# TimingSpace/MVOScaleRecovery

Measured on AMD Instinct MI355X. Metric: frames/sec scale-recovery, KITTI-00 flow (~2k feats/frame), 1/2/4/8 GPU, higher is better.
Workload: dtype f64

## Files before the change

### mvoscalerecovery_amd/csrc/mvosr_kernels.hip

```cpp
#include <hip/hip_runtime.h>
#include <math.h>
#include <stdint.h>
#include <stdlib.h>
#include <string.h>

#include "../../include/mvosr.h"
#include "mvosr_device.hpp"
#include "mvosr_host.hpp"

namespace mvosr {

#ifdef MVOSR_STAMPS
#define MVOSR_STAMP(i) do { if (threadIdx.x == 0 && stamps) stamps[i] = __builtin_amdgcn_s_memtime(); } while (0)
#define MVOSR_STAMP_DECL unsigned long long stamps[12] = {0,0,0,0,0,0,0,0,0,0,0,0};
#define MVOSR_STAMP_ARG , unsigned long long *stamps = nullptr
#define MVOSR_STAMP_PASS , stamps
#define MVOSR_RSTAMP(i) do { if (stamps) stamps[i] = __builtin_amdgcn_s_memtime(); } while (0)
#else
#define MVOSR_RSTAMP(i) do {} while (0)
#define MVOSR_STAMP(i) do {} while (0)
#define MVOSR_STAMP_DECL
#define MVOSR_STAMP_ARG
#define MVOSR_STAMP_PASS
#endif
// ... 519 lines not shown
    double res = 0.0;
    for (int c0 = 0; c0 < n_steep; c0 += kNpBufSize) {
        const int m = min(kNpBufSize, n_steep - c0);
        int k = 0;
        np_pairwise_leaves(m, [&](int lo, int len, bool is_leaf) {
            if (is_leaf) { if (k % B == tid) leaf[k] = np_leaf_sum(hs + c0 + lo, len, 0.0, false); ++k; }
        });
        __threadfence_block();
        __syncthreads();
        if (tid == 0) {
            double val[kNpDepth + 1];
            int vp = 0, kk = 0;
            np_pairwise_leaves(m, [&](int, int, bool is_leaf) {
                if (is_leaf) val[vp++] = leaf[kk++];
                else { const double r = val[--vp], l = val[--vp]; val[vp++] = l + r; }
            });
            *slot = c0 == 0 ? val[0] : *slot + val[0];
        }
        __syncthreads();
    }
    res = *slot;
    __syncthreads();
    return (0.0 + res) / (double)n_steep;
}

struct LdsFetch {
    const double2 *P; const double *Y; int n_valid;
    __device__ __forceinline__ bool operator()(const TriIds q, double &x0, double &y0, double &z0, double &x1, double &y1, double &z1,
                                               double &x2, double &y2, double &z2) const {
        if ((unsigned)q.a >= (unsigned)n_valid || (unsigned)q.b >= (unsigned)n_valid || (unsigned)q.c >= (unsigned)n_valid) return false;
        const double2 p0 = p_ld(P, Y, q.a), p1 = p_ld(P, Y, q.b), p2 = p_ld(P, Y, q.c);
        x0 = p0.x; z0 = p0.y; x1 = p1.x; z1 = p1.y; x2 = p2.x; z2 = p2.y;
        y0 = Y[q.a]; y1 = Y[q.b]; y2 = Y[q.c];
        return true;
    }
};

constexpr double kLevelGuard = 1e-12;

template <int WAVES, int MODE, int FW = 1>
__device__ __forceinline__ SelectResult phase_select(const Smem &s, int n_valid, const int32_t *tri2, int64_t t2_begin,
                                                     int t2_count, TriChunk<WAVES * kWave> &tc, PitchTest pt,
                                                     double *g_normals, double *g_pitch, double *g_heights, int bad_in,
                                                     double *scratch, int scratch_cap, int dbg = 0 MVOSR_STAMP_ARG) {
    constexpr int B = WAVES * kWave;
    constexpr bool FULL = MODE == MODE_FULL;
    const int tid = threadIdx.x;
    unsigned long long flat = 0ull;
    unsigned long long flat_hi = 0ull;
    double hsum = 0.0, hcnt = 0.0, habs = 0.0;
    int npitch = 0, singular = 0, bad = 0;
    int undecided = 0;
    if (t2_count > 64 * FW * B) { bad = 1; t2_count = 0; }
    auto test_triangle = [&](int t, int kk, const TriIds q) {
    if ((unsigned)q.a >= (unsigned)n_valid || (unsigned)q.b >= (unsigned)n_valid || (unsigned)q.c >= (unsigned)n_valid) { bad = 1; return; }
    const double2 p0 = p_ld(s.P, s.Y, q.a), p1 = p_ld(s.P, s.Y, q.b), p2 = p_ld(s.P, s.Y, q.c);
    const double y0 = s.Y[q.a], y1 = s.Y[q.b], y2 = s.Y[q.c];
    const double x0 = p0.x, z0 = p0.y, x1 = p1.x, z1 = p1.y, x2 = p2.x, z2 = p2.y;
    const double h = MODE == MODE_HOT ? (y0 + y1) + y2 : div3((y0 + y1) + y2);
    const int r = classify_triangle<FULL>(x0, y0, z0, x1, y1, z1, x2, y2, z2, h, pt, g_normals, g_pitch, g_heights, t2_begin + t);
    const bool is_flat = r & 1, is_steep = r & 2;
    if (r & 4) singular = 1;
    if constexpr (MODE == MODE_HOT) { if (r & 8) undecided = 1; }
    if (is_steep) { hsum += h; hcnt += 1.0; if constexpr (MODE == MODE_HOT) habs += fabs(h); }
    if (is_flat) {
        if (FW == 1 || kk < 64) flat |= 1ull << (kk & 63); else flat_hi |= 1ull << (kk & 63);
        ++npitch;
    }
    };
    const int t2c = (dbg & 2) ? 0 : t2_count;
    TriChunk<B> tn;
    for (int base = 0; base < t2c; base += kTC * B) {
        const bool more = base + kTC * B < t2c;
        if (more) tn.load(tri2, t2_begin, t2_count, base + kTC * B, tid);
#pragma unroll
        for (int k = 0; k < kTC; ++k) {
            const int t = base + k * B + tid;
            if (t < t2c) test_triangle(t, base / B + k, tc.q[k]);
        }
        if (more) tc = tn;
    }
    const int t2d = (dbg & 4) ? 0 : t2_count;
    const bool in_regs = t2_count <= kTC * B;
    if (!in_regs && t2d > 0) tc.template load<true>(tri2, t2_begin, t2_count, 0, tid);
    if constexpr (MODE == MODE_HOT) block_sum3<WAVES>(hsum, hcnt, habs, s.red + R_SEL_H * 2 * WAVES, s.red + R_SEL_ABS * 2 * WAVES);
    else block_sum2<WAVES>(hsum, hcnt, s.red + R_SEL_H * 2 * WAVES);
    MVOSR_STAMP(4);
    SelectResult r;
    double hl = hsum / hcnt;
    const double guard = kLevelGuard * (habs / hcnt);
    if constexpr (MODE != MODE_HOT) {
        if (scratch && (int)hcnt + kNpMaxLeaves <= scratch_cap)
            hl = exact_height_level_block<WAVES, FULL>(tri2 + 3 * t2_begin, t2_count, (int)hcnt, pt, LdsFetch{s.P, s.Y, n_valid}, nullptr,
                                                       scratch, s.misc + M_WCNT, s.red + R_MISC * 2 * WAVES);
        else
            hl = exact_height_level<FULL>(tri2 + 3 * t2_begin, t2_count, (int)hcnt, pt, LdsFetch{s.P, s.Y, n_valid});
    }
    int ntv = 0, near = undecided;
    auto mark_triangle = [&](int kk, int qa, int qb, int qc) {
        const unsigned long long fw = (FW == 1 || kk < 64) ? flat : flat_hi;
        if (!((fw >> (kk & 63)) & 1ull)) return;
        const double y0 = s.Y[qa], y1 = s.Y[qb], y2 = s.Y[qc];
        const double h = MODE == MODE_HOT ? (y0 + y1) + y2 : div3((y0 + y1) + y2);
        if constexpr (MODE == MODE_HOT) { if (fabs(h - hl) <= guard) near = 1; }
        if (h > hl) {
            ++ntv;
            atomicOr(&s.sel[qa >> 5], 1u << (qa & 31));
            atomicOr(&s.sel[qb >> 5], 1u << (qb & 31));
            atomicOr(&s.sel[qc >> 5], 1u << (qc & 31));
        }
    };
    for (int base = 0; base < t2d; base += kTC * B) {
        const bool more = base + kTC * B < t2d;
        if (more) tn.template load<true>(tri2, t2_begin, t2_count, base + kTC * B, tid);
#pragma unroll
        for (int k = 0; k < kTC; ++k) {
            if (base + k * B + tid < t2d) mark_triangle(base / B + k, tc.q[k].a, tc.q[k].b, tc.q[k].c);
        }
        if (more) tc = tn;
    }
    bad |= bad_in;
    int sn = singular | (near << 16);
    block_sum4i<WAVES>(npitch, ntv, sn, bad, s.red + R_SEL_CNT * 2 * WAVES);
    singular = sn & 0xFFFF;
    r.near = sn >> 16;
    MVOSR_STAMP(5);
    r.height_level = MODE == MODE_HOT ? hl / 3.0 : hl;
    r.n_steep = (int)hcnt;
    r.n_pitch = npitch; r.n_tri_valid = ntv; r.singular = singular; r.bad = bad;
    return r;
}

struct RoadResult {
    double height;
    int status;
    int n_sel, n_kept, n_modes, mode_left, mode_right;
    double mean, std, skew, median;
};

__device__ __forceinline__ bool dropped_by_single(double y, int bin, const Bits192 &single, int first_single) {
    bool d = false;
#pragma unroll
    for (int dk = -1; dk <= 1; ++dk) {
        const int k = bin + dk;
        const bool is_single = (k >= 0) && (k < kBins) && single.test_lane(max(k, 0));
        const double r = bin_edge(k + 1);
        const double lo = r - 0.1;
        const bool in = (k == first_single) ? (y >= lo && y <= r) : (y > lo && y <= r);
        d |= is_single && in;
    }
    return d;
}

#ifndef MVOSR_ROAD_RC
#define MVOSR_ROAD_RC 20
#endif
constexpr int kRoadRC = MVOSR_ROAD_RC;
constexpr int kDropStride = 32;
constexpr int kRoadWaves = 4;
constexpr int kTrash = 175;
constexpr int kStPending = -1;
constexpr int kStRedo = -2;
static_assert(kStRedo == MVOSR_ST_REDO, "include/mvosr.h");
constexpr int kMaxVoteRows = 32765;

struct RoadArgs {
    mvosr_params P;
    const int64_t *off;
    const int32_t *cnt;
    const double *y;
    double *scratch;
    const double *height_level;
    mvosr_outputs o;
    int64_t first_frame, n_frames;
    int pending_only;
    int32_t *level_redo;
    const int32_t *list;
    int wide;
    const uint8_t *listed_mask = nullptr;
};

__device__ __forceinline__ int bin_of_table(double y, const double2 *edges) {
    if (!(y >= 0.0 && y <= bin_edge(kBins))) return -1;
    int k = min((int)(y * 10.0), kBins - 1);
    const double2 e = edges[k];
    k += (k < kBins - 1 && y >= e.y) ? 1 : 0;
    k -= (y < e.x) ? 1 : 0;
    return k;
}

template <int RC, int WW = 1>
__device__ __forceinline__ RoadResult road_wave(int *hist, int *nearflag, uint16_t *slots, uint8_t *dropb, const double2 *edges,
                                                const double *yv_all, double *scratch,
                                                int Mall, double height_level, const mvosr_params &P, int32_t *g_hist, bool exact_stats,
                                                int part_lo, int part_hi, double *part, int *np_stack MVOSR_STAMP_ARG) {
    const int lane = lane_id();
    RoadResult R;
    R.height = nan(""); R.status = MVOSR_ST_MODE; R.n_sel = Mall; R.n_kept = 0; R.n_modes = 0; R.mode_left = -1; R.mode_right = -1;
    R.mean = R.std = R.skew = R.median = nan("");
    if (Mall == 0) { R.status = MVOSR_ST_NO_FLAT; return R; }
    const double *yv = yv_all + (part_hi > part_lo ? part_lo : 0);
    const int M = part_hi - part_lo;
    if (WW == 1 || wave_id() == 0) {
#pragma unroll
        for (int c = 0; c < 3; ++c) { const int b = lane + 64 * c; if (b < 176) hist[b] = 0; }
    }
    if constexpr (WW > 1) __syncthreads();

    double yc[RC];
    int binc[RC];
    const int nfull = M / kWave;
    const unsigned valid = (nfull >= RC) ? (unsigned)((1ull << RC) - 1ull)
                                              : (((1u << nfull) - 1u) | ((lane < M - nfull * kWave ? 1u : 0u) << nfull));
#pragma unroll
    for (int k = 0; k < RC; ++k) {
        const int i = max(min(k * kWave + lane, M - 1), 0);
        yc[k] = yv[i];
    }
#pragma unroll
    for (int k = 0; k < RC; ++k) {
        const double y = yc[k];
        const bool inr = ((valid >> k) & 1u) && (y >= 0.0) && (y <= bin_edge(kBins));
        const int g = inr ? min((int)(y * 10.0), kBins - 1) : 0;
        const double2 e = edges[g];
        int bin = g + ((g < kBins - 1 && y >= e.y) ? 1 : 0) - ((y < e.x) ? 1 : 0);
        bin = inr ? bin : kTrash;
        atomicAdd(&hist[bin], 1);
        binc[k] = bin;
    }
    constexpr int kLongUnroll = 8;
    for (int i0 = RC * kWave + lane; i0 < M; i0 += kLongUnroll * kWave) {
        double yl[kLongUnroll];
#pragma unroll
        for (int j = 0; j < kLongUnroll; ++j) yl[j] = yv[max(min(i0 + j * kWave, M - 1), 0)];
#pragma unroll
        for (int j = 0; j < kLongUnroll; ++j) {
            const int bin = (i0 + j * kWave < M) ? bin_of_table(yl[j], edges) : -1;
            if (bin >= 0) atomicAdd(&hist[bin], 1);
        }
    }
    MVOSR_RSTAMP(2);
    if constexpr (WW > 1) __syncthreads();
    int hraw[3], hz[3];
    Bits192 single, modes, mins;
    int mx = 0, mn = 0x7fffffff;
#pragma unroll
    for (int c = 0; c < 3; ++c) {
        const int b = lane + 64 * c;
        hraw[c] = (b < kBins) ? hist[b] : 0;
        hz[c] = (hraw[c] == 1) ? 0 : hraw[c];
        single.w[c] = __ballot(b < kBins && hraw[c] == 1);
        mx = max(mx, hz[c]);
        if (b < kBins) mn = min(mn, hz[c]);
    }
    mx = wave_max(mx);
    mn = wave_min(mn);
    if (g_hist && (WW == 1 || wave_id() == 0)) {
#pragma unroll
        for (int c = 0; c < 3; ++c) { const int b = lane + 64 * c; if (b < kBins) { g_hist[b] = hraw[c]; g_hist[kBins + b] = hz[c]; } }
    }
    MVOSR_RSTAMP(3);
    const int first_single = single.lowest_from(0);
    Bits192 near;
    near.w[0] = single.w[0] | (single.w[0] << 1) | (single.w[0] >> 1) | (single.w[1] << 63);
    near.w[1] = single.w[1] | (single.w[1] << 1) | (single.w[1] >> 1) | (single.w[0] >> 63) | (single.w[2] << 63);
    near.w[2] = single.w[2] | (single.w[2] << 1) | (single.w[2] >> 1) | (single.w[1] >> 63);
#pragma unroll
    for (int c = 0; c < 3; ++c) { const int b = lane + 64 * c; if (b < 176) nearflag[b] = (b < kBins) ? (int)((near.w[c] >> lane) & 1ull) : 0; }
    const bool have_modes = mx > P.mode_min;

    unsigned kept = valid;
    {
        uint4 zero; zero.x = zero.y = zero.z = zero.w = 0u;
        reinterpret_cast<uint4 *>(dropb)[2 * lane] = zero;
        if (RC > 16) reinterpret_cast<uint4 *>(dropb)[2 * lane + 1] = zero;
        int ns = 0;
#pragma unroll
        for (int k = 0; k < RC; ++k) {
            const bool sus = nearflag[binc[k]] != 0;
            const unsigned long long m = __ballot(sus);
            if (sus) slots[ns + __popcll(m & ((1ull << lane) - 1ull))] = (uint16_t)(k * kWave + lane);
            ns += __popcll(m);
        }
        for (int i = lane; i < ns; i += kWave) {
            const int e = slots[i];
            const double y = yv[e];
            if (dropped_by_single(y, bin_of_table(y, edges), single, first_single)) dropb[(e & (kWave - 1)) * kDropStride + (e >> 6)] = 1;
        }
        if (ns > 0) {
#pragma unroll
            for (int j = 0; j < (RC + 15) / 16; ++j) {
                const uint4 d = reinterpret_cast<const uint4 *>(dropb)[2 * lane + j];
#pragma unroll
                for (int k = 16 * j; k < RC && k < 16 * j + 16; ++k) {
                    const int kk = k & 15;
                    const unsigned w = (kk >> 2) == 0 ? d.x : ((kk >> 2) == 1 ? d.y : ((kk >> 2) == 2 ? d.z : d.w));
                    if ((w >> (8 * (kk & 3))) & 0xFFu) kept &= ~(1u << k);
                }
            }
        }
    }
    double sum = 0.0;
#pragma unroll
    for (int k = 0; k < RC; ++k) sum += ((kept >> k) & 1u) ? yc[k] : 0.0;
    double cntd = (double)__popc(kept);
    for (int i0 = RC * kWave + lane; i0 < M; i0 += kLongUnroll * kWave) {
        double yl[kLongUnroll];
#pragma unroll
        for (int j = 0; j < kLongUnroll; ++j) yl[j] = yv[max(min(i0 + j * kWave, M - 1), 0)];
#pragma unroll
        for (int j = 0; j < kLongUnroll; ++j) {
            if (i0 + j * kWave >= M) continue;
            const double y = yl[j];
            const int bin = bin_of_table(y, edges);
            if (bin >= 0 && nearflag[bin] && dropped_by_single(y, bin, single, first_single)) continue;
            sum += y; cntd += 1.0;
        }
    }
    sum = wave_sum(sum);
    cntd = wave_sum(cntd);
    if constexpr (WW > 1) {
        if (lane == 0) { part[2 * wave_id()] = sum; part[2 * wave_id() + 1] = cntd; }
        __syncthreads();
        sum = 0.0; cntd = 0.0;
#pragma unroll
        for (int i = 0; i < WW; ++i) { sum += part[2 * i]; cntd += part[2 * i + 1]; }
        __syncthreads();
    }
    MVOSR_RSTAMP(4);
    const int nkept = (int)cntd;
    R.n_kept = nkept;

    auto pack_kept = [&]() {
        int nlist = 0;
#pragma unroll 1
        for (int i0 = 0; i0 < Mall; i0 += kWave) {
            const int i = i0 + lane;
            bool keep = false;
            double y = 0.0;
            if (i < Mall) {
                y = yv_all[i];
                const int bin = bin_of_table(y, edges);
                keep = !(bin >= 0 && nearflag[bin] && dropped_by_single(y, bin, single, first_single));
            }
            const unsigned long long m = __ballot(keep);
            if (keep) scratch[nlist + __popcll(m & ((1ull << lane) - 1ull))] = y;
            nlist += __popcll(m);
        }
        return nlist;
    };

    if (!have_modes) {
        if constexpr (WW > 1) { if (wave_id() != 0) return R; }
        if (nkept == 0) { R.height = height_level; R.status = MVOSR_ST_LEVEL; return R; }
        pack_kept();
        __threadfence_block();
        const int klo = (nkept - 1) >> 1, khi = nkept >> 1;
        double mlo = 0.0, mhi = 0.0;
        int flo = 0, fhi = 0;
        for (int i = lane; i < nkept; i += kWave) {
            const double yi = scratch[i];
            int rank = 0;
            for (int j = 0; j < nkept; ++j) {
                const double yj = scratch[j];
                rank += (yj < yi) || (yj == yi && j < i);
            }
            if (rank == klo) { mlo = yi; flo = 1; }
            if (rank == khi) { mhi = yi; fhi = 1; }
        }
        const unsigned long long blo = __ballot(flo), bhi = __ballot(fhi);
        mlo = readlane_d(mlo, (int)__ffsll((long long)blo) - 1);
        mhi = readlane_d(mhi, (int)__ffsll((long long)bhi) - 1);
        R.median = (klo == khi) ? mlo : (mlo + mhi) / 2.0;
        R.height = R.median; R.status = MVOSR_ST_MEDIAN;
        return R;
    }

    const double mean = sum / cntd;
    double ss = 0.0;
#pragma unroll
    for (int k = 0; k < RC; ++k) {
        const double d = ((kept >> k) & 1u) ? yc[k] - mean : 0.0;
        ss += d * d;
    }
    for (int i0 = RC * kWave + lane; i0 < M; i0 += kLongUnroll * kWave) {
        double yl[kLongUnroll];
#pragma unroll
        for (int j = 0; j < kLongUnroll; ++j) yl[j] = yv[max(min(i0 + j * kWave, M - 1), 0)];
#pragma unroll
        for (int j = 0; j < kLongUnroll; ++j) {
            if (i0 + j * kWave >= M) continue;
            const double y = yl[j];
            const int bin = bin_of_table(y, edges);
            if (bin >= 0 && nearflag[bin] && dropped_by_single(y, bin, single, first_single)) continue;
            const double d = y - mean;
            ss += d * d;
        }
    }
    ss = wave_sum(ss);
    if constexpr (WW > 1) {
        if (lane == 0) part[wave_id()] = ss;
        __syncthreads();
        if (wave_id() != 0) return R;
        ss = 0.0;
#pragma unroll
        for (int i = 0; i < WW; ++i) ss += part[i];
    }
    MVOSR_RSTAMP(5);

#pragma unroll
    for (int c = 0; c < 3; ++c) {
        const int b = lane + 64 * c;
        bool is_mode = false, is_min = false;
        if (b < kBins) {
            const int h = hz[c];
            if (b == 0 || b == kBins - 1) {
                is_mode = (h == mx);
                is_min = (h == mn);
            } else {
                const int lraw = hist[b - 1], rraw = hist[b + 1];
                const int hl_ = (lraw == 1) ? 0 : lraw, hr_ = (rraw == 1) ? 0 : rraw;
                is_mode = (h >= hl_) && (h >= hr_) && ((double)h >= P.mode_rel * (double)mx) && (h >= P.mode_min);
                is_min = (h <= hl_) && (h <= hr_) && !((h == hr_) && (h == hl_));
            }
        }
        modes.w[c] = __ballot(is_mode);
        mins.w[c] = __ballot(is_min);
    }
    R.n_modes = modes.runs();
    const int i_last = modes.highest_below(kBins);
    int i_first = i_last;
    while (i_first > 0 && modes.test(i_first - 1)) --i_first;
    const int ml = i_first + 1, mr = i_last + 1;
    R.mode_left = ml; R.mode_right = mr;
    const double mode = (double)(ml + mr) / 2.0;
    const int il = mins.highest_below(ml);
    if (il < 0) { R.status = MVOSR_ST_ERR_LEFT; return R; }
    const int ir = mins.lowest_from(mr);
    if (ir < 0) { R.status = MVOSR_ST_ERR_RIGHT; return R; }
    const double right = bin_edge(ir + 1);
    double mean_o = mean;
    double sd = sqrt(ss / cntd);
    {
        const double var = ss / cntd, rms = sqrt(mean * mean + var);
        const double margin = fabs((mean - mode / 10.0) - P.skew_threshold * sd);
        const double bound = 1e-11 * (rms + sd) + 1e-22 * rms * rms / sd;
        if (!(margin > bound) || exact_stats) {
            const int nl = pack_kept();
            __threadfence_block();
            mean_o = np_pairwise_sum_cold(scratch, nl, 0.0, 0, np_stack) / (double)nl;
            sd = sqrt(np_pairwise_sum_cold(scratch, nl, mean_o, 1, np_stack) / (double)nl);
        }
    }
    const double skew = (mean_o - mode / 10.0) / sd;
    R.mean = mean_o; R.std = sd; R.skew = skew;
    if (skew > P.skew_threshold) { R.height = right; R.status = MVOSR_ST_RIGHT; }
    else { R.height = mode / 10.0; R.status = MVOSR_ST_MODE; }
    return R;
}

#ifndef MVOSR_ROAD_MINW
#define MVOSR_ROAD_MINW 1
#endif
template <bool LIST, int WW = 1>
__global__ __launch_bounds__(kRoadWaves *kWave, (LIST ? 1 : 4)) void road_model_kernel(const RoadArgs a) {
    static_assert(kRoadRC >= 16 && kRoadRC <= kDropStride, "verdict bytes per lane; the keep masks are 32 bits");
    static_assert(WW == 1 || (WW == kRoadWaves && !LIST), "wide variant: the whole workgroup on one frame");
    __shared__ int hist_all[kRoadWaves][2][176];
    __shared__ double2 edges[kBins + 1];
    __shared__ uint16_t slots_all[kRoadWaves][kRoadRC * kWave];
    __shared__ __attribute__((aligned(16))) uint8_t drop_all[kRoadWaves][kDropStride * kWave];
    __shared__ double part[2 * kRoadWaves];
    __shared__ __attribute__((aligned(8))) int np_stack_all[kRoadWaves][kNpStackInts];
    for (int k = threadIdx.x; k < kBins; k += kRoadWaves * kWave) { double2 e; e.x = bin_edge(k); e.y = bin_edge(k + 1); edges[k] = e; }
    __syncthreads();
    const int64_t slot = WW > 1 ? (int64_t)blockIdx.x : (int64_t)blockIdx.x * kRoadWaves + wave_id();
    auto one_frame = [&](const int64_t f) {
    if (a.pending_only && a.o.status[f] != kStPending) return;
    MVOSR_STAMP_DECL
    MVOSR_RSTAMP(0);
    const int M = a.cnt[f];
    const int64_t off = a.off[f];
    const double hl = a.height_level ? a.height_level[f] : nan("");
    MVOSR_RSTAMP(1);
    int *h0 = hist_all[WW > 1 ? 0 : wave_id()][0], *h1 = hist_all[wave_id()][1];
    int32_t *gh = a.o.hist ? a.o.hist + f * 2 * kBins : nullptr;
    const bool ex = a.o.stats != nullptr;
    int lo = 0, hi = M;
    if constexpr (WW > 1) {
        const int q = ((M + WW * kWave - 1) / (WW * kWave)) * kWave;
        lo = min(M, wave_id() * q);
        hi = min(M, lo + q);
    }
    const int Mp = hi - lo;
#define MVOSR_ROAD_CALL(RC_) road_wave<RC_, WW>(h0, h1, slots_all[wave_id()], drop_all[wave_id()], edges, a.y + off, a.scratch + off, M, hl, a.P, gh, ex, lo, hi, part, np_stack_all[wave_id()] MVOSR_STAMP_PASS)
    const RoadResult R = (Mp <= 4 * kWave) ? MVOSR_ROAD_CALL(4)
                       : (Mp <= 8 * kWave) ? MVOSR_ROAD_CALL(8)
                       : (Mp <= 12 * kWave) ? MVOSR_ROAD_CALL(12)
                       : (kRoadRC == 16 || Mp <= 16 * kWave) ? MVOSR_ROAD_CALL(16)
                                          : MVOSR_ROAD_CALL(kRoadRC);
#undef MVOSR_ROAD_CALL
    MVOSR_RSTAMP(6);
#ifdef MVOSR_STAMPS
    if (lane_id() == 0 && a.o.hist) { unsigned long long *d = reinterpret_cast<unsigned long long *>(a.o.hist + f * 2 * kBins) + 16; for (int i = 0; i < 8; ++i) d[i] = stamps[i]; }
#endif
    if (WW > 1 && wave_id() != 0) return;
    if (R.status == MVOSR_ST_LEVEL && a.level_redo) {
        if (lane_id() == 0) {
            if (!(a.listed_mask && a.listed_mask[f])) a.level_redo[1 + atomicAdd(a.level_redo, 1)] = (int32_t)f;
            a.o.status[f] = kStRedo;
        }
        return;
    }
    if (lane_id() == 0) {
        double height = nan(""), raw = nan("");
        if (R.status == MVOSR_ST_NO_FLAT) raw = a.P.absolute_reference / hl;
        else if (R.status <= MVOSR_ST_LEVEL) { height = R.height; raw = a.P.absolute_reference / height; }
        a.o.raw_scale[f] = raw; a.o.height[f] = height; a.o.status[f] = R.status;
        if (!a.pending_only && a.o.height_level) a.o.height_level[f] = hl;
        if (a.o.counts) {
            int32_t *c = a.o.counts + f * MVOSR_N_COUNTS;
            if (!a.pending_only) { c[MVOSR_CNT_VALID] = M; c[MVOSR_CNT_TRI_PITCH] = 0; c[MVOSR_CNT_TRI_VALID] = 0; }
            c[MVOSR_CNT_SELECTED] = R.n_sel; c[MVOSR_CNT_KEPT] = R.n_kept; c[MVOSR_CNT_MODES] = R.n_modes;
            c[MVOSR_CNT_MODE_LEFT] = R.mode_left; c[MVOSR_CNT_MODE_RIGHT] = R.mode_right;
        }
        if (a.o.stats) { double *st = a.o.stats + 4 * f; st[0] = R.mean; st[1] = R.std; st[2] = R.skew; st[3] = R.median; }
    }
    };
    if constexpr (LIST) {
        const int64_t n_todo = (int64_t)a.list[0];
        for (int64_t it = slot; it < n_todo; it += (int64_t)gridDim.x * kRoadWaves) one_frame((int64_t)a.list[1 + it]);
    } else {
        if (slot < a.n_frames) one_frame(a.first_frame + slot);
    }
}

struct KArgs {
    mvosr_params P;
    mvosr_batch b;
    mvosr_outputs o;
    PitchTest pt;
    int64_t first_frame;
    const double *height_level_in;
    int debug_skip;
    int32_t *redo;
    int redo_pass;
    double *ysel;
    int32_t *nsel;
    const int32_t *cls_list;
    const int32_t *cls_cnt;
};

__device__ __forceinline__ void write_counts(const KArgs &a, int64_t f, int nvalid, int npitch, int ntv, const RoadResult &R) {
    if (!a.o.counts) return;
    int32_t *c = a.o.counts + f * MVOSR_N_COUNTS;
    c[MVOSR_CNT_VALID] = nvalid; c[MVOSR_CNT_TRI_PITCH] = npitch; c[MVOSR_CNT_TRI_VALID] = ntv;
    c[MVOSR_CNT_SELECTED] = R.n_sel; c[MVOSR_CNT_KEPT] = R.n_kept; c[MVOSR_CNT_MODES] = R.n_modes;
    c[MVOSR_CNT_MODE_LEFT] = R.mode_left; c[MVOSR_CNT_MODE_RIGHT] = R.mode_right;
}

__device__ __forceinline__ bool early_frame_exit(const KArgs &a, int64_t f, int n, int t2n) {
    const bool too_few = n == 3;
    const bool oversize = n > a.b.max_feat;
    if (!(n <= 2 || too_few || t2n <= 0 || oversize)) return false;
    if (threadIdx.x == 0) {
        RoadResult R;
        R.n_sel = R.n_kept = R.n_modes = 0; R.mode_left = R.mode_right = -1;
        a.o.raw_scale[f] = nan(""); a.o.height[f] = nan(""); a.o.height_level[f] = nan("");
        a.o.status[f] = oversize ? MVOSR_ST_ERR_MASK : (too_few ? MVOSR_ST_TOO_FEW : MVOSR_ST_ERR_EMPTY);
        a.nsel[f] = 0;
        write_counts(a, f, too_few ? n : 0, 0, 0, R);
    }
    return true;
}

template <int BW, int MODE>
__device__ __forceinline__ void frame_tail(const KArgs &a, const Smem &s, int64_t f, int64_t off, int nvalid, bool refused,
                                           SelectResult &S, RoadResult &R) {
    constexpr int B = BW * kWave;
    const int tid = threadIdx.x;
    int status = kStPending;
    double raw = nan("");
    int nsel = 0;
    if (refused || S.bad) {
        status = MVOSR_ST_ERR_MASK;
    } else if (S.singular) {
        status = MVOSR_ST_ERR_SINGULAR;
    } else {
        const int w = wave_id(), lane = lane_id();
        const int per = ((nvalid + B - 1) / B) * kWave;
        const int begin = w * per, end = min(nvalid, begin + per);
        int cnt = 0;
        for (int j0 = begin; j0 < end; j0 += kWave) {
            const int j = j0 + lane;
            const bool sel = (j < end) && ((s.sel[j >> 5] >> (j & 31)) & 1u);
            if (a.o.selected && j < end) a.o.selected[off + j] = (uint8_t)sel;
            cnt += __popcll(__ballot(sel));
        }
        if (lane == 0) s.misc[M_WCNT + w] = cnt;
        __syncthreads();
        int base = 0;
#pragma unroll
        for (int i = 0; i < BW; ++i) { const int c = s.misc[M_WCNT + i]; if (i < w) base += c; nsel += c; }
        if constexpr (MODE == MODE_HOT) {
            if (S.near || nsel == 0) {
                if (tid == 0) { a.redo[1 + atomicAdd(a.redo, 1)] = (int32_t)f; a.o.status[f] = kStRedo; a.nsel[f] = 0; }
                return;
            }
        }
        double *dst = a.ysel + off;
        for (int j0 = begin; j0 < end; j0 += kWave) {
            const int j = j0 + lane;
            const bool sel = (j < end) && ((s.sel[j >> 5] >> (j & 31)) & 1u);
            const unsigned long long m = __ballot(sel);
            if (sel) dst[base + __popcll(m & ((1ull << lane) - 1ull))] = s.Y[j];
            base += __popcll(m);
        }
        if (nsel == 0) { status = MVOSR_ST_NO_FLAT; raw = a.P.absolute_reference / S.height_level; }
    }
    if (tid == 0) {
        a.o.raw_scale[f] = raw;
        a.o.height[f] = nan("");
        a.o.height_level[f] = S.height_level;
        a.o.status[f] = status;
        a.nsel[f] = nsel;
        R.n_sel = nsel;
        write_counts(a, f, nvalid, S.n_pitch, S.n_tri_valid, R);
        if (a.o.stats) { double *st = a.o.stats + 4 * f; st[0] = st[1] = st[2] = st[3] = nan(""); }
    }
}

template <int MODE, bool LIST, class Body>
__device__ __forceinline__ void for_frames(const KArgs &a, Body body) {
    if constexpr (MODE == MODE_EXACT) {
        if (a.redo_pass) {
            const int count = a.redo[0];
            for (int i = blockIdx.x; i < count; i += gridDim.x) {
                body((int64_t)a.redo[1 + i]);
                __syncthreads();
            }
            return;
        }
    }
    if constexpr (LIST) {
        if ((int)blockIdx.x < *a.cls_cnt) body((int64_t)a.cls_list[blockIdx.x]);
        return;
    }
    body(a.first_frame + blockIdx.x);
}

#ifndef MVOSR_MINW
#define MVOSR_MINW 1
// ... 1290 lines not shown
        if ((rc = launch_append_mask(ctx, ka, n_launch, false))) return rc;
        if (standin && (rc = standin_rows(ka.redo))) return rc;
        if ((rc = dense ? launch_scale_dense(ctx, ka, n_launch, kModeExactList, false) : dispatch_scale(ctx, ka, waves, n_launch, kModeExactList))) return rc;
        ra.first_frame = first_frame; ra.n_frames = n_launch; ra.list = ka.redo;
        ra.wide = (dense && !(debug_skip_env() & 256)) ? 1 : 0;
        return launch_road(ctx, ra, ctx_stream(ctx));
    }
    const bool fold = mode == MODE_HOT && (hot_only || (!(debug_skip_env() & 16) && !(debug_skip_env() & 512)));
    if (by_class) {
        if ((rc = launch_scale_classes(ctx, ka, n_launch))) return rc;
        if (!hot_only && (rc = launch_append_mask(ctx, ka, n_launch, true))) return rc;
        if (!fold && (rc = dispatch_scale(ctx, ka, waves, n_launch, kModeExactList))) return rc;
    } else {
        g_defer_exact = fold;
        g_hot_only = hot_only;
        rc = dense ? launch_scale_dense(ctx, ka, n_launch, mode, false) : dispatch_scale(ctx, ka, waves, n_launch, mode);
        g_defer_exact = false;
        g_hot_only = false;
        if (rc) return rc;
    }
    if (pev && (ee = hipEventRecord(pev[1], ctx_stream(ctx))) != hipSuccess) return set_hip_error("hipEventRecord(profile)", ee);
    ra.first_frame = first_frame; ra.n_frames = n_launch;
    ra.wide = (dense && !(debug_skip_env() & 256)) ? 1 : 0;
    if (!(debug_skip_env() & 16)) {
        if (fold) {
            ra.level_redo = ka.redo;
            ra.listed_mask = hot_only ? nullptr : b->exact_mask;
            if ((rc = launch_road(ctx, ra, ctx_stream(ctx)))) return rc;
            ra.listed_mask = nullptr;
            if (hot_only) return MVOSR_OK;
            if (standin && (rc = standin_rows(ka.redo))) return rc;
            if ((rc = dense ? launch_scale_dense(ctx, ka, n_launch, kModeExactList, false) : dispatch_scale(ctx, ka, waves, n_launch, kModeExactList))) return rc;
            ra.level_redo = nullptr; ra.list = ka.redo;
            if ((rc = launch_road(ctx, ra, ctx_stream(ctx)))) return rc;
        } else {
            if (mode == MODE_HOT) {
                const hipError_t e2 = hipMemsetAsync(redo2, 0, sizeof(int32_t), ctx_stream(ctx));
                if (e2 != hipSuccess) return set_hip_error("hipMemsetAsync(redo list 2)", e2);
                ra.level_redo = redo2;
            }
            if ((rc = launch_road(ctx, ra, ctx_stream(ctx)))) return rc;
            if (mode == MODE_HOT) {
                KArgs k2 = ka;
                k2.redo = redo2;
                if ((rc = dense ? launch_scale_dense(ctx, k2, n_launch, kModeExactList, false) : dispatch_scale(ctx, k2, waves, n_launch, kModeExactList))) return rc;
                ra.level_redo = nullptr; ra.list = redo2;
                if ((rc = launch_road(ctx, ra, ctx_stream(ctx)))) return rc;
            }
        }
    }
    if (pev) {
        if ((ee = hipEventRecord(pev[2], ctx_stream(ctx))) != hipSuccess) return set_hip_error("hipEventRecord(profile)", ee);
        ctx->prof_calls++;
    }
    return MVOSR_OK;
}

int mvosr_batch_size_hint(const int32_t *feat_cnt_host, int64_t n_frames, mvosr_batch *b) {
    if (!b || n_frames < 0 || (n_frames > 0 && !feat_cnt_host)) return set_error(MVOSR_ERR_ARG, "batch_size_hint: null argument");
    int64_t cnt[3] = {0, 0, 0};
    int32_t lo = 0, hi = 0;
    for (int64_t f = 0; f < n_frames; ++f) {
        const int32_t n = feat_cnt_host[f];
        if (n < 0) return set_error(MVOSR_ERR_ARG, "batch_size_hint: negative feature count");
        if (f == 0 || n < lo) lo = n;
        if (f == 0 || n > hi) hi = n;
        ++cnt[size_class_of(n)];
    }
    b->max_feat = hi;
    b->min_feat = lo;
    for (int c = 0; c < 3; ++c) b->size_hint[c] = (int32_t)(cnt[c] > 0x7fffffff ? 0x7fffffff : cnt[c]);
    b->size_hint[3] = kClassHintMagic;
    return MVOSR_OK;
}

int mvosr_outlier_vote_batch(mvosr_ctx *ctx, const mvosr_params *p, const mvosr_batch *b, const mvosr_outputs *o,
                             int waves_per_frame) {
    int rc = check_common(ctx, p, b, o);
    if (rc) return rc;
    if (!b->y || !b->z || !b->v || !b->tri1_off || !b->tri1) return set_error(MVOSR_ERR_ARG, "outlier_vote: missing y/z/v/tri1");
    if (!o->vote_counters) return set_error(MVOSR_ERR_ARG, "outlier_vote: vote_counters output required");
    if (b->n_frames == 0) return MVOSR_OK;
    if ((rc = ctx_activate(ctx))) return rc;
    KArgs ka;
    ka.P = *p; ka.b = *b; ka.o = *o; ka.pt = make_pitch_test(p->pitch_threshold_deg);
    ka.first_frame = 0; ka.height_level_in = nullptr; ka.debug_skip = 0; ka.ysel = nullptr; ka.nsel = nullptr; ka.redo = nullptr; ka.redo_pass = 0;
    ka.cls_list = nullptr; ka.cls_cnt = nullptr;
    if ((waves_per_frame == 0 || waves_per_frame == 16) && b->max_feat > lds_capacity_features()) {
        if (b->total_feat <= 0) return set_error(MVOSR_ERR_ARG, "outlier_vote: batch.total_feat not set");
        return launch_scale_dense(ctx, ka, b->n_frames, MODE_HOT, true);
    }
    return dispatch_vote(ctx, ka, pick_waves(waves_per_frame, b->max_feat), b->n_frames);
}

int mvosr_road_model_batch(mvosr_ctx *ctx, const mvosr_params *p, const mvosr_batch *b, const double *height_level_in,
                           const mvosr_outputs *o, int waves_per_frame) {
    (void)waves_per_frame;
    int rc = check_common(ctx, p, b, o);
    if (rc) return rc;
    if (!b->y) return set_error(MVOSR_ERR_ARG, "road_model: y plane required");
    if (!o->raw_scale || !o->height || !o->status) return set_error(MVOSR_ERR_ARG, "road_model: raw_scale/height/status required");
    if (b->n_frames == 0) return MVOSR_OK;
    if (b->total_feat <= 0) return set_error(MVOSR_ERR_ARG, "road_model: batch.total_feat (length of the y plane) not set");
    if ((rc = ctx_activate(ctx))) return rc;
    RoadArgs ra;
    double *scratch = nullptr;
    int32_t *unused = nullptr;
    if ((rc = ctx_workspace(ctx, b->n_frames, b->total_feat, &scratch, &unused))) return rc;
    ra.P = *p; ra.off = b->feat_off; ra.cnt = b->feat_cnt; ra.y = b->y; ra.scratch = scratch;
    ra.height_level = height_level_in; ra.o = *o;
    ra.first_frame = 0; ra.n_frames = b->n_frames; ra.pending_only = 0; ra.level_redo = nullptr; ra.list = nullptr;
    ra.wide = b->max_feat > 4 * kRoadRC * kWave ? 1 : 0;
    return launch_road(ctx, ra, ctx_stream(ctx));
}

static int launch_window_median(mvosr_ctx *ctx, const double *raw, int64_t n, int n_blocks, int64_t stride, int window,
                                const double *queue_in, int n_queue, double *out) {
    if (!ctx || (n > 0 && (!raw || !out))) return set_error(MVOSR_ERR_ARG, "window_median: null argument");
    if (window < 1 || window > kMaxWindow) return set_error(MVOSR_ERR_ARG, "window_median: window must be in 1..%d", kMaxWindow);
    if (n_queue < 0 || n_queue > window || (n_queue > 0 && !queue_in)) return set_error(MVOSR_ERR_ARG, "window_median: bad carried-in queue");
    if (n_blocks < 1) return set_error(MVOSR_ERR_ARG, "window_median: n_blocks < 1");
    if (n <= 0) return MVOSR_OK;
    MedianArgs ma;
    ma.raw = raw; ma.out = out; ma.n = n; ma.window = window; ma.n_queue = n_queue;
    ma.n_blocks = n_blocks; ma.base_len = n / n_blocks; ma.extra = n % n_blocks; ma.stride = stride;
    if (n_blocks > 1 && stride < ma.base_len + (ma.extra ? 1 : 0)) return set_error(MVOSR_ERR_ARG, "window_median: block stride shorter than a block");
    int rc = ctx_activate(ctx);
    if (rc) return rc;
    for (int i = 0; i < kMaxWindow; ++i) ma.queue[i] = (i < n_queue) ? queue_in[i] : 0.0;
    hipLaunchKernelGGL(window_median_kernel, dim3((unsigned)((n + 255) / 256)), dim3(256), 0, ctx_stream(ctx), ma);
    return check_launch("window_median_kernel");
}

int mvosr_window_median(mvosr_ctx *ctx, const double *raw, int64_t n, int window, const double *queue_in, int n_queue,
                        double *out) {
    return launch_window_median(ctx, raw, n, 1, 0, window, queue_in, n_queue, out);
}

int mvosr_window_median_blocked(mvosr_ctx *ctx, const double *blocks, int64_t n, int n_blocks, int64_t block_stride, int window,
                                const double *queue_in, int n_queue, double *out) {
    return launch_window_median(ctx, blocks, n, n_blocks, block_stride, window, queue_in, n_queue, out);
}

}

#ifdef MVOSR_ABLATE
extern "C" int mvosr_debug_redo_list(mvosr_ctx *ctx, int64_t n_frames, int32_t *out, int cap) {
    if (!ctx || !out || cap < 1 || !ctx->ws_nsel) return MVOSR_ERR_ARG;
    (void)hipStreamSynchronize(ctx_stream(ctx));
    const hipError_t e = hipMemcpy(out, ctx->ws_nsel + n_frames, sizeof(int32_t) * (size_t)cap, hipMemcpyDeviceToHost);
    return e == hipSuccess ? MVOSR_OK : MVOSR_ERR_HIP;
}
#endif
```

Baseline: 25.83 million.

## Fuse road stats into a single shifted-moment pass with sub-histograms

The road-model kernel now computes the mean and variance in one pass using shifted sums and sum-of-squares. Dropped samples' contributions are subtracted afterwards instead of running a separate keep pass and a second variance pass. The shared histogram is split into four lane sub-histograms to cut atomic contention, bins are packed into registers instead of slot and drop buffers, and the exact-fallback error bound is widened to cover the one-pass rounding. It also cuts LDS use, raises the launch-bounds occupancy hint to 6, and adds an RC=20 dispatch. The trade-off is a wider error band that may send more frames to the exact fallback, plus some numeric risk from the one-pass variance.

```diff
diff --git a/mvoscalerecovery_amd/csrc/mvosr_kernels.hip b/mvoscalerecovery_amd/csrc/mvosr_kernels.hip
--- a/mvoscalerecovery_amd/csrc/mvosr_kernels.hip
+++ b/mvoscalerecovery_amd/csrc/mvosr_kernels.hip
@@ -695,11 +695,14 @@
     return d;
 }
 
+#ifdef MVOSR_ROAD_EXACT_COUNT
+__device__ unsigned long long g_road_exact_count[3];
+#endif
 #ifndef MVOSR_ROAD_RC
 #define MVOSR_ROAD_RC 20
 #endif
 constexpr int kRoadRC = MVOSR_ROAD_RC;
-constexpr int kDropStride = 32;
+constexpr int kRoadSub = 4;
 constexpr int kRoadWaves = 4;
 constexpr int kTrash = 175;
 constexpr int kStPending = -1;
@@ -733,10 +736,11 @@
 }
 
 template <int RC, int WW = 1>
-__device__ __forceinline__ RoadResult road_wave(int *hist, int *nearflag, uint16_t *slots, uint8_t *dropb, const double2 *edges,
+__device__ __forceinline__ RoadResult road_wave(int *hist, int *comb, uint8_t *nearflag, const double2 *edges,
                                                 const double *yv_all, double *scratch,
                                                 int Mall, double height_level, const mvosr_params &P, int32_t *g_hist, bool exact_stats,
                                                 int part_lo, int part_hi, double *part, int *np_stack MVOSR_STAMP_ARG) {
+    static_assert(RC <= 32 && kRoadSub == 4, "32-bit row masks; one int4 per bin");
     const int lane = lane_id();
     RoadResult R;
     R.height = nan(""); R.status = MVOSR_ST_MODE; R.n_sel = Mall; R.n_kept = 0; R.n_modes = 0; R.mode_left = -1; R.mode_right = -1;
@@ -745,41 +749,57 @@
     const double *yv = yv_all + (part_hi > part_lo ? part_lo : 0);
     const int M = part_hi - part_lo;
     if (WW == 1 || wave_id() == 0) {
-#pragma unroll
-        for (int c = 0; c < 3; ++c) { const int b = lane + 64 * c; if (b < 176) hist[b] = 0; }
+        int4 z; z.x = z.y = z.z = z.w = 0;
+#pragma unroll
+        for (int c = 0; c < 3; ++c) { const int b = lane + 64 * c; if (b < 176) reinterpret_cast<int4 *>(hist)[b] = z; }
     }
     if constexpr (WW > 1) __syncthreads();
-
-    double yc[RC];
-    int binc[RC];
+    const double y0 = yv_all[0];
+    const double sh = (y0 - y0 == 0.0) ? y0 : 0.0;
+    int *hsub = hist + (lane & (kRoadSub - 1));
+
     const int nfull = M / kWave;
     const unsigned valid = (nfull >= RC) ? (unsigned)((1ull << RC) - 1ull)
                                               : (((1u << nfull) - 1u) | ((lane < M - nfull * kWave ? 1u : 0u) << nfull));
-#pragma unroll
-    for (int k = 0; k < RC; ++k) {
-        const int i = max(min(k * kWave + lane, M - 1), 0);
-        yc[k] = yv[i];
-    }
-#pragma unroll
-    for (int k = 0; k < RC; ++k) {
-        const double y = yc[k];
-        const bool inr = ((valid >> k) & 1u) && (y >= 0.0) && (y <= bin_edge(kBins));
-        const int g = inr ? min((int)(y * 10.0), kBins - 1) : 0;
-        const double2 e = edges[g];
-        int bin = g + ((g < kBins - 1 && y >= e.y) ? 1 : 0) - ((y < e.x) ? 1 : 0);
-        bin = inr ? bin : kTrash;
-        atomicAdd(&hist[bin], 1);
-        binc[k] = bin;
-    }
-    constexpr int kLongUnroll = 8;
+    double s1 = 0.0, s2 = 0.0;
+    unsigned pk[(RC + 3) / 4];
+    constexpr int kG = 4;
+#pragma unroll
+    for (int k0 = 0; k0 < RC; k0 += kG) {
+        double yg[kG];
+#pragma unroll
+        for (int j = 0; j < kG && k0 + j < RC; ++j) yg[j] = yv[max(min((k0 + j) * kWave + lane, M - 1), 0)];
+#pragma unroll
+        for (int j = 0; j < kG && k0 + j < RC; ++j) {
+            const int k = k0 + j;
+            const double y = yg[j];
+            const bool vk = (valid >> k) & 1u;
+            const bool inr = vk && (y >= 0.0) && (y <= bin_edge(kBins));
+            const int g = inr ? min((int)(y * 10.0), kBins - 1) : 0;
+            const double2 e = edges[g];
+            int bin = g + ((g < kBins - 1 && y >= e.y) ? 1 : 0) - ((y < e.x) ? 1 : 0);
+            bin = inr ? bin : kTrash;
+            atomicAdd(&hsub[4 * bin], 1);
+            const double d = vk ? y - sh : 0.0;
+            s1 += d;
+            s2 = __builtin_fma(d, d, s2);
+            pk[k >> 2] = (k & 3) ? (pk[k >> 2] | ((unsigned)bin << (8 * (k & 3)))) : (unsigned)bin;
+        }
+        __builtin_amdgcn_sched_barrier(0);
+    }
+    constexpr int kLongUnroll = 2;
     for (int i0 = RC * kWave + lane; i0 < M; i0 += kLongUnroll * kWave) {
         double yl[kLongUnroll];
 #pragma unroll
         for (int j = 0; j < kLongUnroll; ++j) yl[j] = yv[max(min(i0 + j * kWave, M - 1), 0)];
 #pragma unroll
         for (int j = 0; j < kLongUnroll; ++j) {
-            const int bin = (i0 + j * kWave < M) ? bin_of_table(yl[j], edges) : -1;
-            if (bin >= 0) atomicAdd(&hist[bin], 1);
+            if (i0 + j * kWave >= M) continue;
+            const int bin = bin_of_table(yl[j], edges);
+            if (bin >= 0) atomicAdd(&hsub[4 * bin], 1);
+            const double d = yl[j] - sh;
+            s1 += d;
+            s2 = __builtin_fma(d, d, s2);
         }
     }
     MVOSR_RSTAMP(2);
@@ -790,7 +810,10 @@
 #pragma unroll
     for (int c = 0; c < 3; ++c) {
         const int b = lane + 64 * c;
-        hraw[c] = (b < kBins) ? hist[b] : 0;
+        int h = 0;
+        if (b < kBins) { const int4 q = reinterpret_cast<const int4 *>(hist)[b]; h = (q.x + q.y) + (q.z + q.w); }
+        if (b < 176) comb[b] = h;
+        hraw[c] = h;
         hz[c] = (hraw[c] == 1) ? 0 : hraw[c];
         single.w[c] = __ballot(b < kBins && hraw[c] == 1);
         mx = max(mx, hz[c]);
@@ -809,44 +832,27 @@
     near.w[1] = single.w[1] | (single.w[1] << 1) | (single.w[1] >> 1) | (single.w[0] >> 63) | (single.w[2] << 63);
     near.w[2] = single.w[2] | (single.w[2] << 1) | (single.w[2] >> 1) | (single.w[1] >> 63);
 #pragma unroll
-    for (int c = 0; c < 3; ++c) { const int b = lane + 64 * c; if (b < 176) nearflag[b] = (b < kBins) ? (int)((near.w[c] >> lane) & 1ull) : 0; }
+    for (int c = 0; c < 3; ++c) { const int b = lane + 64 * c; if (b < 176) nearflag[b] = (b < kBins) ? (uint8_t)((near.w[c] >> lane) & 1ull) : 0; }
     const bool have_modes = mx > P.mode_min;
 
-    unsigned kept = valid;
+    double t1 = 0.0, t2 = 0.0;
+    int nd = 0;
     {
-        uint4 zero; zero.x = zero.y = zero.z = zero.w = 0u;
-        reinterpret_cast<uint4 *>(dropb)[2 * lane] = zero;
-        if (RC > 16) reinterpret_cast<uint4 *>(dropb)[2 * lane + 1] = zero;
-        int ns = 0;
-#pragma unroll
-        for (int k = 0; k < RC; ++k) {
-            const bool sus = nearflag[binc[k]] != 0;
-            const unsigned long long m = __ballot(sus);
-            if (sus) slots[ns + __popcll(m & ((1ull << lane) - 1ull))] = (uint16_t)(k * kWave + lane);
-            ns += __popcll(m);
-        }
-        for (int i = lane; i < ns; i += kWave) {
-            const int e = slots[i];
-            const double y = yv[e];
-            if (dropped_by_single(y, bin_of_table(y, edges), single, first_single)) dropb[(e & (kWave - 1)) * kDropStride + (e >> 6)] = 1;
-        }
-        if (ns > 0) {
-#pragma unroll
-            for (int j = 0; j < (RC + 15) / 16; ++j) {
-                const uint4 d = reinterpret_cast<const uint4 *>(dropb)[2 * lane + j];
-#pragma unroll
-                for (int k = 16 * j; k < RC && k < 16 * j + 16; ++k) {
-                    const int kk = k & 15;
-                    const unsigned w = (kk >> 2) == 0 ? d.x : ((kk >> 2) == 1 ? d.y : ((kk >> 2) == 2 ? d.z : d.w));
-                    if ((w >> (8 * (kk & 3))) & 0xFFu) kept &= ~(1u << k);
-                }
+        unsigned sus = 0u;
+#pragma unroll
+        for (int k = 0; k < RC; ++k) sus |= (nearflag[(pk[k >> 2] >> (8 * (k & 3))) & 0xFFu] ? 1u : 0u) << k;
+        while (sus) {
+            const int k = __ffs(sus) - 1;
+            sus &= sus - 1u;
+            const double y = yv[k * kWave + lane];
+            if (dropped_by_single(y, bin_of_table(y, edges), single, first_single)) {
+                const double d = y - sh;
+                t1 += d;
+                t2 = __builtin_fma(d, d, t2);
+                ++nd;
             }
         }
     }
-    double sum = 0.0;
-#pragma unroll
-    for (int k = 0; k < RC; ++k) sum += ((kept >> k) & 1u) ? yc[k] : 0.0;
-    double cntd = (double)__popc(kept);
     for (int i0 = RC * kWave + lane; i0 < M; i0 += kLongUnroll * kWave) {
         double yl[kLongUnroll];
 #pragma unroll
@@ -856,22 +862,28 @@
             if (i0 + j * kWave >= M) continue;
             const double y = yl[j];
             const int bin = bin_of_table(y, edges);
-            if (bin >= 0 && nearflag[bin] && dropped_by_single(y, bin, single, first_single)) continue;
-            sum += y; cntd += 1.0;
-        }
-    }
-    sum = wave_sum(sum);
-    cntd = wave_sum(cntd);
+            if (bin >= 0 && nearflag[bin] && dropped_by_single(y, bin, single, first_single)) {
+                const double d = y - sh;
+                t1 += d;
+                t2 = __builtin_fma(d, d, t2);
+                ++nd;
+            }
+        }
+    }
+    double S1 = wave_sum(s1 - t1), S2 = wave_sum(s2 - t2), Q = wave_sum(s2);
+    nd = wave_sum(nd);
     if constexpr (WW > 1) {
-        if (lane == 0) { part[2 * wave_id()] = sum; part[2 * wave_id() + 1] = cntd; }
+        if (lane == 0) { part[4 * wave_id()] = S1; part[4 * wave_id() + 1] = S2; part[4 * wave_id() + 2] = Q; part[4 * wave_id() + 3] = (double)nd; }
         __syncthreads();
-        sum = 0.0; cntd = 0.0;
-#pragma unroll
-        for (int i = 0; i < WW; ++i) { sum += part[2 * i]; cntd += part[2 * i + 1]; }
-        __syncthreads();
+        S1 = 0.0; S2 = 0.0; Q = 0.0;
+        double ndd = 0.0;
+#pragma unroll
+        for (int i = 0; i < WW; ++i) { S1 += part[4 * i]; S2 += part[4 * i + 1]; Q += part[4 * i + 2]; ndd += part[4 * i + 3]; }
+        nd = (int)ndd;
     }
     MVOSR_RSTAMP(4);
-    const int nkept = (int)cntd;
+    const int nkept = Mall - nd;
+    const double cntd = (double)nkept;
     R.n_kept = nkept;
 
     auto pack_kept = [&]() {
@@ -918,37 +930,7 @@
         R.height = R.median; R.status = MVOSR_ST_MEDIAN;
         return R;
     }
-
-    const double mean = sum / cntd;
-    double ss = 0.0;
-#pragma unroll
-    for (int k = 0; k < RC; ++k) {
-        const double d = ((kept >> k) & 1u) ? yc[k] - mean : 0.0;
-        ss += d * d;
-    }
-    for (int i0 = RC * kWave + lane; i0 < M; i0 += kLongUnroll * kWave) {
-        double yl[kLongUnroll];
-#pragma unroll
-        for (int j = 0; j < kLongUnroll; ++j) yl[j] = yv[max(min(i0 + j * kWave, M - 1), 0)];
-#pragma unroll
-        for (int j = 0; j < kLongUnroll; ++j) {
-            if (i0 + j * kWave >= M) continue;
-            const double y = yl[j];
-            const int bin = bin_of_table(y, edges);
-            if (bin >= 0 && nearflag[bin] && dropped_by_single(y, bin, single, first_single)) continue;
-            const double d = y - mean;
-            ss += d * d;
-        }
-    }
-    ss = wave_sum(ss);
-    if constexpr (WW > 1) {
-        if (lane == 0) part[wave_id()] = ss;
-        __syncthreads();
-        if (wave_id() != 0) return R;
-        ss = 0.0;
-#pragma unroll
-        for (int i = 0; i < WW; ++i) ss += part[i];
-    }
+    if constexpr (WW > 1) { if (wave_id() != 0) return R; }
     MVOSR_RSTAMP(5);
 
 #pragma unroll
@@ -961,7 +943,7 @@
                 is_mode = (h == mx);
                 is_min = (h == mn);
             } else {
-                const int lraw = hist[b - 1], rraw = hist[b + 1];
+                const int lraw = comb[b - 1], rraw = comb[b + 1];
                 const int hl_ = (lraw == 1) ? 0 : lraw, hr_ = (rraw == 1) ? 0 : rraw;
                 is_mode = (h >= hl_) && (h >= hr_) && ((double)h >= P.mode_rel * (double)mx) && (h >= P.mode_min);
                 is_min = (h <= hl_) && (h <= hr_) && !((h == hr_) && (h == hl_));
@@ -982,12 +964,28 @@
     const int ir = mins.lowest_from(mr);
     if (ir < 0) { R.status = MVOSR_ST_ERR_RIGHT; return R; }
     const double right = bin_edge(ir + 1);
+    const double m1 = S1 / cntd;
+    const double mean = sh + m1;
+    const double var = S2 / cntd - m1 * m1;
     double mean_o = mean;
-    double sd = sqrt(ss / cntd);
+    double sd = sqrt(var);
     {
-        const double var = ss / cntd, rms = sqrt(mean * mean + var);
+        const double thr = fabs(P.skew_threshold);
+        const double N = (double)Mall;
+        const double g = 0x1p-52 * (2.0 * (double)((Mall + kWave - 1) / kWave) + 64.0 + N / (double)kNpBufSize);
+        const double a2 = Q / cntd, r = sqrt(a2), rho = sqrt(N / cntd), Mg = fabs(sh) + r;
+        const double rms = sqrt(mean * mean + var);
         const double margin = fabs((mean - mode / 10.0) - P.skew_threshold * sd);
-        const double bound = 1e-11 * (rms + sd) + 1e-22 * rms * rms / sd;
+        const double bound_two_pass = 1e-11 * (rms + sd) + 1e-22 * rms * rms / sd;
+        const double bound = bound_two_pass
+                           + g * ((Mg + rho * r) + fabs(mode / 10.0) + (1.0 + thr) * sd + (1.0 + thr) * (a2 * (6.0 + 2.0 * rho) + g * Mg * Mg) / sd);
+#ifdef MVOSR_ROAD_EXACT_COUNT
+        if (lane == 0) {
+            atomicAdd(&g_road_exact_count[0], 1ull);
+            if (!(margin > bound_two_pass)) atomicAdd(&g_road_exact_count[1], 1ull);
+            if (!(margin > bound)) atomicAdd(&g_road_exact_count[2], 1ull);
+        }
+#endif
         if (!(margin > bound) || exact_stats) {
             const int nl = pack_kept();
             __threadfence_block();
@@ -1005,15 +1003,18 @@
 #ifndef MVOSR_ROAD_MINW
 #define MVOSR_ROAD_MINW 1
 #endif
+#ifndef MVOSR_ROAD_OCC
+#define MVOSR_ROAD_OCC 6
+#endif
 template <bool LIST, int WW = 1>
-__global__ __launch_bounds__(kRoadWaves *kWave, (LIST ? 1 : 4)) void road_model_kernel(const RoadArgs a) {
-    static_assert(kRoadRC >= 16 && kRoadRC <= kDropStride, "verdict bytes per lane; the keep masks are 32 bits");
+__global__ __launch_bounds__(kRoadWaves *kWave, (LIST ? 1 : MVOSR_ROAD_OCC)) void road_model_kernel(const RoadArgs a) {
+    static_assert(kRoadRC >= 16 && kRoadRC <= 32, "the row masks are 32 bits");
     static_assert(WW == 1 || (WW == kRoadWaves && !LIST), "wide variant: the whole workgroup on one frame");
-    __shared__ int hist_all[kRoadWaves][2][176];
+    __shared__ __attribute__((aligned(16))) int hist_all[kRoadWaves][kRoadSub * 176];
+    __shared__ int comb_all[kRoadWaves][176];
+    __shared__ uint8_t near_all[kRoadWaves][176];
     __shared__ double2 edges[kBins + 1];
-    __shared__ uint16_t slots_all[kRoadWaves][kRoadRC * kWave];
-    __shared__ __attribute__((aligned(16))) uint8_t drop_all[kRoadWaves][kDropStride * kWave];
-    __shared__ double part[2 * kRoadWaves];
+    __shared__ double part[4 * kRoadWaves];
     __shared__ __attribute__((aligned(8))) int np_stack_all[kRoadWaves][kNpStackInts];
     for (int k = threadIdx.x; k < kBins; k += kRoadWaves * kWave) { double2 e; e.x = bin_edge(k); e.y = bin_edge(k + 1); edges[k] = e; }
     __syncthreads();
@@ -1026,7 +1027,7 @@
     const int64_t off = a.off[f];
     const double hl = a.height_level ? a.height_level[f] : nan("");
     MVOSR_RSTAMP(1);
-    int *h0 = hist_all[WW > 1 ? 0 : wave_id()][0], *h1 = hist_all[wave_id()][1];
+    int *h0 = hist_all[WW > 1 ? 0 : wave_id()];
     int32_t *gh = a.o.hist ? a.o.hist + f * 2 * kBins : nullptr;
     const bool ex = a.o.stats != nullptr;
     int lo = 0, hi = M;
@@ -1036,11 +1037,12 @@
         hi = min(M, lo + q);
     }
     const int Mp = hi - lo;
-#define MVOSR_ROAD_CALL(RC_) road_wave<RC_, WW>(h0, h1, slots_all[wave_id()], drop_all[wave_id()], edges, a.y + off, a.scratch + off, M, hl, a.P, gh, ex, lo, hi, part, np_stack_all[wave_id()] MVOSR_STAMP_PASS)
+#define MVOSR_ROAD_CALL(RC_) road_wave<RC_, WW>(h0, comb_all[wave_id()], near_all[wave_id()], edges, a.y + off, a.scratch + off, M, hl, a.P, gh, ex, lo, hi, part, np_stack_all[wave_id()] MVOSR_STAMP_PASS)
     const RoadResult R = (Mp <= 4 * kWave) ? MVOSR_ROAD_CALL(4)
                        : (Mp <= 8 * kWave) ? MVOSR_ROAD_CALL(8)
                        : (Mp <= 12 * kWave) ? MVOSR_ROAD_CALL(12)
                        : (kRoadRC == 16 || Mp <= 16 * kWave) ? MVOSR_ROAD_CALL(16)
+                       : (kRoadRC <= 20 || Mp <= 20 * kWave) ? MVOSR_ROAD_CALL(kRoadRC <= 20 ? kRoadRC : 20)
                                           : MVOSR_ROAD_CALL(kRoadRC);
 #undef MVOSR_ROAD_CALL
     MVOSR_RSTAMP(6);
@@ -2637,3 +2639,15 @@
     return e == hipSuccess ? MVOSR_OK : MVOSR_ERR_HIP;
 }
 #endif
+
+#ifdef MVOSR_ROAD_EXACT_COUNT
+extern "C" int mvosr_debug_road_exact_count(unsigned long long *out, int reset) {
+    if (hipDeviceSynchronize() != hipSuccess) return MVOSR_ERR_HIP;
+    if (hipMemcpyFromSymbol(out, HIP_SYMBOL(mvosr::g_road_exact_count), 3 * sizeof(unsigned long long)) != hipSuccess) return MVOSR_ERR_HIP;
+    if (reset) {
+        const unsigned long long z[3] = {0ull, 0ull, 0ull};
+        if (hipMemcpyToSymbol(HIP_SYMBOL(mvosr::g_road_exact_count), z, sizeof z) != hipSuccess) return MVOSR_ERR_HIP;
+    }
+    return MVOSR_OK;
+}
+#endif
diff --git a/profiles/road_exact_count.py b/profiles/road_exact_count.py
--- /dev/null
+++ b/profiles/road_exact_count.py
@@ -0,0 +1,19 @@
+#!/usr/bin/env python3
+import ctypes as C
+import os
+import runpy
+import sys
+
+R = os.path.dirname(os.path.dirname(os.path.abspath(__file__)))
+sys.argv = [os.path.join(R, "bench.py"), "--no-cpu-baseline", "--no-e2e"] + sys.argv[1:]
+try:
+    runpy.run_path(sys.argv[0], run_name="__main__")
+except SystemExit as e:
+    if e.code not in (None, 0):
+        raise
+from mvoscalerecovery_amd import _lib
+lib = C.CDLL(_lib.LIB_PATH)
+out = (C.c_ulonglong * 3)()
+assert lib.mvosr_debug_road_exact_count(out, 0) == 0
+n, old, new = out[0], out[1], out[2]
+print("road decisions %d  exact (two-pass band) %d = %.3g  exact (band in use) %d = %.3g" % (n, old, old / max(n, 1), new, new / max(n, 1)))
```

Measured after the change: 26.45 million, median of 6. +2.4%, better.
